# aksiksi/needle

Measured on AMD Instinct MI355X. Metric: episode-pairs/sec (analyze+search), higher is better.
Workload: dtype f64-certified (f32 first pass)

## Files before the change

needle_amd/csrc/search.hip:

```cpp
#include "epilogue.h"
#include "hipctx.h"

#include <algorithm>
#include <atomic>
#include <cstdio>
#include <cstdlib>
#include <cstring>
#include <mutex>
#include <unordered_map>

namespace needle {

namespace {

constexpr int kDiagsPerBlock = 256;
constexpr int kBandR = 7, kBandU = 3;
constexpr int kBandB = 64 * kBandR;
constexpr int kSampleW = 8;
constexpr int kSampleHead = 3;
__host__ __device__ constexpr int head_row(int k, int W, int H = kSampleHead) {
  return H == 3 ? (k == 0 ? 0 : (k == 1 ? W / 2 : W - 1)) : (k * (W - 1)) / (H - 1);
}
__host__ __device__ constexpr bool is_head_row(int s, int W, int H = kSampleHead) {
  for (int k = 0; k < H; k++)
// ... 99 lines not shown
  const int D0 = band * B - (n - 2);
  if (D0 > m - 2) return;
  const int i_start = max(1, 2 - D0 - B);
  const int i_end = min(n - 1, m - 1 - D0);
  if (i_start > i_end) return;
  const int d_l = D0 + lane * R;
  const int min_len = (int)pr.min_len;
  const int flag_len = min_len - K + 1;

  uint32_t W[R];
  int Z[R];
#pragma unroll
  for (int r = 0; r < R; r++) {
    W[r] = lds[B + i_start + d_l + r];
    Z[r] = i_start - 1;
  }

  auto checkpoint = [&](int c) {
#pragma unroll
    for (int r = 0; r < R; r++) {
      if (c - Z[r] >= flag_len) {
        const int d = d_l + r;
        const int ilo = d < 0 ? 1 - d : 1;
        const int ihi = min(n - 1, m - 1 - d);
        if (c >= ilo && c <= ihi) {
          const int a = max(Z[r] + 1, ilo);
          const int limit = min(ihi, c + K);
          int e = c + 1;
          while (e <= limit && (uint32_t)__popc(src[e] ^ lds[B + e + d]) <= threshold) e++;
          const bool reaches_next_checkpoint = (e > limit) && (limit == c + K);
          if (!reaches_next_checkpoint) {
            const int b = e - 1;
            const int len = b - a + 1;
            if (len >= min_len) {
              const uint32_t slot = atomicAdd(count, 1u);
              if (slot < capacity) runs[slot] = NeedleHipRun{(uint32_t)lo, (uint32_t)b, (uint32_t)(b + d), (uint32_t)len, 0u, 0u};
            }
          }
        }
      }
    }
  };

  int i = i_start;
  for (; i + K - 1 <= i_end; i += K) {
    const uint32_t *__restrict__ nxt = lds + (B + i + d_l + R);
#pragma unroll
    for (int s = 0; s < K; s++) {
      const int row = i + s;
      const uint32_t sv = src[row];
#pragma unroll
      for (int r = 0; r < R; r++) {
        const uint32_t c = (uint32_t)__popc(sv ^ W[(r + s) % R]);
        Z[r] = (c <= threshold) ? Z[r] : row;
        if (r == 0) W[s % R] = nxt[s];
      }
    }
    bool any = false;
#pragma unroll
    for (int r = 0; r < R; r++) any |= (i + K - 1 - Z[r] >= flag_len);
    if (__any(any)) checkpoint(i + K - 1);
  }
  for (; i <= i_end; i++) {
    const uint32_t sv = src[i];
#pragma unroll
    for (int r = 0; r < R; r++) {
      const uint32_t c = (uint32_t)__popc(sv ^ W[r]);
      Z[r] = (c <= threshold) ? Z[r] : i;
    }
#pragma unroll
    for (int r = 0; r + 1 < R; r++) W[r] = W[r + 1];
    W[R - 1] = lds[B + i + d_l + R];
  }
}

__device__ __forceinline__ void wave_lds_fence_search() {
  __builtin_amdgcn_fence(__ATOMIC_RELEASE, "wavefront");
  __builtin_amdgcn_wave_barrier();
  __builtin_amdgcn_fence(__ATOMIC_ACQUIRE, "wavefront");
}

template <int R, int W, bool COUNT = false, int H = kSampleHead, bool LEGACY = false>
__global__ __launch_bounds__(256) void hamming_runs_sampled_kernel(const uint32_t *__restrict__ hashes,
                                                                   const SearchProblem *__restrict__ problems,
                                                                   int num_problems, uint32_t threshold,
                                                                   NeedleHipRun *__restrict__ runs,
                                                                   uint32_t capacity, uint32_t *__restrict__ count,
                                                                   int bands_per_wave, int sparse_max,
                                                                   unsigned long long *__restrict__ eval_groups) {
  constexpr int B = 64 * R;
  unsigned long long groups = 0, survived = 0;
  extern __shared__ uint32_t lds[];
  __builtin_amdgcn_s_setprio(3);
  int lo = 0, hi = num_problems - 1;
  while (lo < hi) {
    int mid = (lo + hi + 1) >> 1;
    if (problems[mid].block_base <= blockIdx.x) lo = mid; else hi = mid - 1;
  }
  const SearchProblem pr = problems[lo];
  const int n = (int)pr.n, m = (int)pr.m;
  const uint32_t *__restrict__ src = hashes + pr.src_off;
  const uint32_t *__restrict__ dst = hashes + pr.dst_off;
  uint32_t *ldst = lds;
  for (int k = threadIdx.x; k < B; k += blockDim.x) {
    ldst[k] = 0u;
    ldst[B + m + k] = 0u;
  }
  {
    constexpr int kU = 8;
    const int nt = (int)blockDim.x;
    int k = threadIdx.x;
    for (; k + (kU - 1) * nt < m; k += kU * nt) {
      uint32_t v[kU];
#pragma unroll
      for (int u = 0; u < kU; u++) v[u] = dst[k + u * nt];
#pragma unroll
      for (int u = 0; u < kU; u++) ldst[B + k + u * nt] = v[u];
    }
    for (; k < m; k += nt) ldst[B + k] = dst[k];
  }
  const uint32_t *__restrict__ lsrc = src;
  __syncthreads();

  const int wave = __builtin_amdgcn_readfirstlane((int)(threadIdx.x >> 6));
  const int lane = (int)(threadIdx.x & 63);
  const int min_len = (int)pr.min_len;
  const int P = min_len - W + 1;
  const uint32_t bias = 31u - min(threshold, 31u);
  uint32_t held_b = 0u, held_e = 0u, held_len = 0u;
  int held = 0;
  auto flush_runs = [&]() {
    if (held == 0) return;
    uint32_t base = 0u;
    if (lane == 0) base = atomicAdd(count, (uint32_t)held);
    base = (uint32_t)__builtin_amdgcn_readfirstlane((int)base);
    if (lane < held && base + (uint32_t)lane < capacity)
      runs[base + (uint32_t)lane] = NeedleHipRun{(uint32_t)lo, held_b, held_e, held_len, 0u, 0u};
    held = 0;
  };
  auto emit_run = [&](const uint32_t b, const uint32_t e, const uint32_t len) {
    const bool mine = lane == held;
    held_b = mine ? b : held_b;
    held_e = mine ? e : held_e;
    held_len = mine ? len : held_len;
    if (++held == 64) flush_runs();
  };
  const int slots = 4 * bands_per_wave;
  const int total_bands = (n + m - 3 + B - 1) / B;
  const int nb = (total_bands + slots - 1) / slots;
  const int b_in_pair = (int)(blockIdx.x - pr.block_base);
  for (int round = 0; round < bands_per_wave; round++) {
  const int q = (round * 4 + wave + lo) % slots;
  const int band = q * nb + b_in_pair;
  const int D0 = band * B - (n - 2);
  if (band >= total_bands || D0 > m - 2) continue;
  const int i_start = max(1, 2 - D0 - B);
  const int i_end = min(n - 1, m - 1 - D0);
  const int d_l = D0 + lane * R;

  int k0 = (i_start - 1 + P - 1) / P;
  for (int w0 = 1 + k0 * P; w0 + W - 1 <= i_end; w0 += P) {
    uint32_t E[W + R - 1];
#pragma unroll
    for (int q = 0; q < W + R - 1; q++) E[q] = ldst[B + w0 + d_l + q];
    uint32_t sv[W];
#pragma unroll
    for (int s = 0; s < W; s++) sv[s] = src[w0 + s];
    bool ok[R];
    uint32_t miss[R];
#pragma unroll
    for (int r = 0; r < R; r++) miss[r] = 0u;
#pragma unroll
    for (int k = 0; k < H; k++) {
      const int s = head_row(k, W, H);
#pragma unroll
      for (int r = 0; r < R; r++) miss[r] |= (uint32_t)__popc(sv[s] ^ E[s + r]) + bias;
    }
#pragma unroll
    for (int r = 0; r < R; r++) ok[r] = miss[r] < 32u;
    if (COUNT) groups += H * R;
    auto resolve = [&](const int d) {
      const int ilo = d < 0 ? 1 - d : 1;
      const int ihi = min(n - 1, m - 1 - d);
      if (w0 < ilo || w0 + W - 1 > ihi) return;
      int e = w0 + W;
      bool ended = false;
      const int fwd_limit = min(ihi, w0 + P + W - 1);
      while (e <= fwd_limit) {
        const int row = e + lane;
        const bool bad = row <= fwd_limit && (uint32_t)__popc(lsrc[row] ^ ldst[B + row + d]) > threshold;
        if (COUNT) groups += 1;
        const unsigned long long mm = __ballot(bad);
        if (mm) {
          e += __ffsll((long long)mm) - 1;
          ended = true;
          break;
        }
        e += 64;
      }
      if (!ended) {
        if (fwd_limit == w0 + P + W - 1) return;
        e = ihi + 1;
      }
      const int b = e - 1;
      int a = ilo;
      int q = w0 - 1;
      while (q >= ilo) {
        const int row = q - lane;
        const bool bad = row >= ilo && (uint32_t)__popc(lsrc[row] ^ ldst[B + row + d]) > threshold;
        if (COUNT) groups += 1;
        const unsigned long long mm = __ballot(bad);
        if (mm) {
          a = q - (__ffsll((long long)mm) - 1) + 1;
          break;
        }
        q -= 64;
      }
      const int len = b - a + 1;
      if (len >= min_len) emit_run((uint32_t)b, (uint32_t)(b + d), (uint32_t)len);
    };

    unsigned long long alive[R];
    int survivors = 0;
#pragma unroll
    for (int r = 0; r < R; r++) {
      alive[r] = __ballot(ok[r]);
      survivors += __popcll(alive[r]);
    }
    if (COUNT) survived += (unsigned long long)survivors;
    if (survivors == 0) continue;
    if (!LEGACY || sparse_max < 0) {
#pragma unroll
      for (int r = 0; r < R; r++) {
        if (alive[r] == 0) continue;
        uint32_t mm = miss[r];
#pragma unroll
        for (int k = 0; k < W - H; k++) {
          const int s = tail_row(k, W, H);
          mm |= (uint32_t)__popc(sv[s] ^ E[s + r]) + bias;
        }
        if (COUNT) groups += W - H;
        unsigned long long cand = __ballot(mm < 32u);
        while (cand) {
          const int src_lane = __ffsll((long long)cand) - 1;
          cand &= cand - 1;
          resolve(D0 + src_lane * R + r);
        }
      }
      continue;
    }
    if constexpr (LEGACY) {
    if (survivors <= sparse_max) {
      constexpr int kTail = W - H;
      uint32_t sv_tail = sv[tail_row(kTail - 1, W, H)];
      int tail_off = tail_row(kTail - 1, W, H);
#pragma unroll
      for (int k = kTail - 2; k >= 0; k--) {
        sv_tail = lane == k ? sv[tail_row(k, W, H)] : sv_tail;
        tail_off = lane == k ? tail_row(k, W, H) : tail_off;
      }
#pragma unroll
      for (int r = 0; r < R; r++) {
        unsigned long long cand = alive[r];
        while (cand) {
          const int src_lane = __ffsll((long long)cand) - 1;
          cand &= cand - 1;
          const int d = D0 + src_lane * R + r;
          const int row = w0 + tail_off;
          const bool bad = (uint32_t)__popc(sv_tail ^ ldst[B + row + d]) > threshold;
          if (COUNT) groups += 1;
          if (__ballot(bad) == 0) resolve(d);
        }
      }
      continue;
    }
#pragma unroll
    for (int k = 0; k < W - H; k++) {
      const int s = tail_row(k, W, H);
#pragma unroll
      for (int r = 0; r < R; r++) miss[r] |= (uint32_t)__popc(sv[s] ^ E[s + r]) + bias;
    }
#pragma unroll
    for (int r = 0; r < R; r++) ok[r] = miss[r] < 32u;
    if (COUNT) groups += (W - H) * R;
#pragma unroll
    for (int r = 0; r < R; r++) {
      unsigned long long cand = __ballot(ok[r]);
      while (cand) {
        const int src_lane = __ffsll((long long)cand) - 1;
        cand &= cand - 1;
        resolve(D0 + src_lane * R + r);
      }
    }
    }
  }
  }
  flush_runs();
  if (COUNT && lane == 0) {
    atomicAdd(eval_groups, groups);
    atomicAdd(eval_groups + 1, survived);
  }
}

__host__ __device__ constexpr int mfma_windows(int n, int min_len, int W) {
  return (n - 1 - W) >= 0 && min_len - W + 1 > 0 ? (n - 1 - W) / (min_len - W + 1) + 1 : 0;
}
typedef int mfma_v4i __attribute__((ext_vector_type(4)));
typedef int mfma_v8i __attribute__((ext_vector_type(8)));
typedef float mfma_v16f __attribute__((ext_vector_type(16)));

#include "scan_mfma_kernel.h"

struct TransposeLane {
  uint32_t rot[5], mask[5];
};
__device__ __forceinline__ TransposeLane transpose_lane(uint32_t lane) {
  TransposeLane t;
  uint32_t m = 0x0000FFFFu;
#pragma unroll
  for (int k = 0; k < 5; k++) {
    const uint32_t j = 16u >> k;
    const bool hi = (lane & j) != 0u;
    t.rot[k] = hi ? 32u - j : j;
    t.mask[k] = hi ? m << j : m;
    m ^= m << (j >> 1);
  }
  return t;
}
template <int PATTERN>
__device__ __forceinline__ uint32_t swizzle_xor(uint32_t x) {
  return (uint32_t)__builtin_amdgcn_ds_swizzle((int)x, PATTERN);
}
__device__ __forceinline__ uint32_t transpose32(uint32_t x, const TransposeLane &t) {
#define NEEDLE_TSTEP(K, J)                                                              \
  {                                                                                     \
    const uint32_t y = swizzle_xor<((J) << 10) | 0x1F>(x);                              \
    const uint32_t r = __builtin_amdgcn_alignbit(y, y, t.rot[K]);                      \
    x = (r & t.mask[K]) | (x & ~t.mask[K]);                                             \
  }
  NEEDLE_TSTEP(0, 16) NEEDLE_TSTEP(1, 8) NEEDLE_TSTEP(2, 4) NEEDLE_TSTEP(3, 2) NEEDLE_TSTEP(4, 1)
#undef NEEDLE_TSTEP
  return x;
}
__device__ __forceinline__ uint32_t wave_simhash32(const uint32_t *__restrict__ slice, uint32_t count, uint32_t lane, const TransposeLane &t) {
  constexpr int kBlocks = 8;
  uint32_t ones = 0;
  for (uint32_t q0 = 0; q0 < count; q0 += 64 * kBlocks) {
    uint32_t h[kBlocks];
#pragma unroll
    for (int u = 0; u < kBlocks; u++) {
      const uint32_t q = q0 + 64 * u + lane;
      h[u] = q < count ? slice[q] : 0u;
    }
#pragma unroll
    for (int u = 0; u < kBlocks; u++) {
      if (q0 + 64 * u >= count) break;
      ones += (uint32_t)__popc(transpose32(h[u], t));
    }
  }
  ones += (uint32_t)__shfl_xor((int)ones, 32);
  const unsigned long long set = __builtin_amdgcn_ballot_w64(2u * ones > count);
  return __brev((uint32_t)set);
}

__global__ __launch_bounds__(256) void simhash_runs_kernel(const uint32_t *__restrict__ hashes,
                                                           const SearchProblem *__restrict__ problems,
                                                           NeedleHipRun *__restrict__ runs, uint32_t capacity,
                                                           const uint32_t *__restrict__ count) {
  const uint32_t total = min(*count, capacity);
  const uint32_t wave = (blockIdx.x * blockDim.x + threadIdx.x) >> 6, waves = (gridDim.x * blockDim.x) >> 6;
  const uint32_t lane = threadIdx.x & 63;
  __builtin_amdgcn_s_setprio(3);
  const TransposeLane t = transpose_lane(lane);
  for (uint32_t k = wave; k < total; k += waves) {
    const NeedleHipRun r = runs[k];
    const SearchProblem pr = problems[r.problem];
    const uint32_t src_hash = wave_simhash32(hashes + pr.src_off + (r.src_end - r.len), r.len + 1u, lane, t);
    const uint32_t dst_hash = wave_simhash32(hashes + pr.dst_off + (r.dst_end - r.len), r.len + 1u, lane, t);
    if (lane == 0) {
      runs[k].problem = pr.tag;
      runs[k].src_match_hash = src_hash;
      runs[k].dst_match_hash = dst_hash;
    }
  }
}

struct ScanShape {
  int w = kSampleW, h = kSampleHead;
};
ScanShape scan_shape() {
  ScanShape sh;
  if (const char *e = getenv("NEEDLE_HIP_SCAN_SHAPE")) {
    int w = 0, h = 0;
    if (std::sscanf(e, "%d,%d", &w, &h) == 2 && (w == 4 || w == 8 || w == 16) && h >= 2 && h <= 4 && h < w) {
      sh.w = w;
      sh.h = h;
    }
  }
  return sh;
}
using SampledKernel = void (*)(const uint32_t *, const SearchProblem *, int, uint32_t, NeedleHipRun *, uint32_t, uint32_t *, int, int,
                               unsigned long long *);
template <bool COUNT>
SampledKernel sampled_kernel(ScanShape sh, bool legacy) {
#define NEEDLE_SHAPE(W_, H_) \
  if (sh.w == W_ && sh.h == H_) return hamming_runs_sampled_kernel<kBandR, W_, COUNT, H_, true>;
  NEEDLE_SHAPE(4, 2) NEEDLE_SHAPE(4, 3) NEEDLE_SHAPE(8, 2) NEEDLE_SHAPE(8, 4) NEEDLE_SHAPE(16, 2) NEEDLE_SHAPE(16, 3) NEEDLE_SHAPE(16, 4)
#undef NEEDLE_SHAPE
  if (legacy) return hamming_runs_sampled_kernel<kBandR, kSampleW, COUNT, kSampleHead, true>;
  return hamming_runs_sampled_kernel<kBandR, kSampleW, COUNT, kSampleHead, false>;
}

struct SearchPlan {
  std::vector<NeedleHipSeq> seqs;
  std::vector<NeedleHipProblem> problems;
  int mode[8] = {0, 0, 0, 0, 0, 0, 0, 0};
  std::vector<SearchProblem> meta;
  size_t staged = 0;
  uint64_t oversize_blocks = 0;
  uint64_t blocks = 0;
  size_t lds_bytes = 0;
  bool sampled = false, fast = false, mfma = false;
  int mfma_waves = 0, mfma_splits = 1;
  std::vector<M2ImageSeq> image_seqs;
  uint32_t image_windows = 0, image_min_len = 0;
  uint64_t mfma_products = 0;
  int bands_per_wave = 1;
  bool valid = false;
  bool matches(const NeedleHipSeq *s, size_t ns, const NeedleHipProblem *p, size_t np, const int *m) const {
    return valid && seqs.size() == ns && problems.size() == np && std::memcmp(mode, m, sizeof(mode)) == 0 &&
           std::memcmp(seqs.data(), s, ns * sizeof(NeedleHipSeq)) == 0 &&
           std::memcmp(problems.data(), p, np * sizeof(NeedleHipProblem)) == 0;
  }
};

int device_cus() {
  int cus = 256, dev = 0;
  if (hipGetDevice(&dev) == hipSuccess) (void)hipDeviceGetAttribute(&cus, hipDeviceAttributeMultiprocessorCount, dev);
  return cus > 0 ? cus : 256;
}

Status build_plan(const NeedleHipSeq *seqs, size_t num_seqs, const NeedleHipProblem *problems, size_t num_problems,
                  const int *mode, SearchPlan *plan) {
  plan->valid = false;
  std::vector<SearchProblem> &meta = plan->meta;
  meta.clear();
  meta.reserve(num_problems);
  uint64_t blocks = 0;
  for (size_t p = 0; p < num_problems; p++) {
    const NeedleHipProblem &pr = problems[p];
    if (pr.src_seq >= num_seqs || pr.dst_seq >= num_seqs)
      return Status::Make(NeedleError_InvalidArgument, "hamming_runs: problem references a missing sequence");
    if (pr.min_len == 0) return Status::Make(NeedleError_InvalidArgument, "hamming_runs: min_len must be >= 1");
    const NeedleHipSeq &a = seqs[pr.src_seq], &b = seqs[pr.dst_seq];
    if (a.len < 2 || b.len < 2) continue;
    SearchProblem m;
    m.src_off = a.offset;
    m.n = a.len;
    m.dst_off = b.offset;
    m.m = b.len;
    m.min_len = pr.min_len;
    m.tag = pr.tag;
    m.block_base = 0;
    m.pad = 0;
    meta.push_back(m);
  }
  plan->staged = 0;
  plan->oversize_blocks = 0;
  if (!meta.empty()) {
    uint32_t smallest = 0xFFFFFFFFu;
    for (const SearchProblem &m : meta) smallest = std::min(smallest, m.min_len);
    const bool generic_only = mode[0] != 0;
    const bool sampled = !generic_only && smallest >= (uint32_t)(2 * scan_shape().w - 1 + 8) && mode[1] == 0 && mode[3] == 0;
    const bool fast = !generic_only && !sampled && smallest >= (uint32_t)(kBandR * kBandU);
    const size_t lds_limit = (size_t)mode[5];
    auto windows_of = [&](const SearchProblem &m) { return (uint64_t)mfma_windows((int)m.n, (int)m.min_len, kSampleW); };
    auto same_group = [](const SearchProblem &a, const SearchProblem &b) {
      return a.dst_off == b.dst_off && a.m == b.m && a.min_len == b.min_len;
    };
    const int waves = mode[6];
    const size_t group_budget = waves == 4 ? 53760 : waves == 8 ? 81920 : 163840;
    const size_t max_members = (size_t)kM2Members;
    auto group_need = [&](const SearchProblem &a, uint64_t windows) { return m2_lds_words(a.m, windows, waves) * sizeof(uint32_t); };
    bool mfma = sampled && mode[4] == 1;
    const size_t mfma_from = 2048;
    const bool candidate = sampled && (mode[4] == 1 || (mode[4] == 2 && meta.size() >= mfma_from));
    if (candidate) {
      std::stable_sort(meta.begin(), meta.end(), [](const SearchProblem &a, const SearchProblem &b) {
        if (a.dst_off != b.dst_off) return a.dst_off < b.dst_off;
        if (a.m != b.m) return a.m < b.m;
        return a.min_len < b.min_len;
      });
      if (!mfma) {
        uint64_t windows = 0, rows = 0;
        for (size_t i = 0; i < meta.size(); i++) {
          uint64_t w = windows_of(meta[i]);
          for (size_t k = 1; k < max_members && i + 1 < meta.size() && same_group(meta[i], meta[i + 1]) &&
                             group_need(meta[i], w + windows_of(meta[i + 1])) <= group_budget; k++)
            w += windows_of(meta[++i]);
          windows += w;
          rows += (w + 31) / 32 * 32;
        }
        mfma = rows > 0 && 10 * windows >= 7 * rows;
      }
    }
    auto lds_need = [&](const SearchProblem &m) {
      if (mfma) return group_need(m, windows_of(m));
      return ((fast || sampled) ? (size_t)m.m + 2 * kBandB : (size_t)m.n + m.m) * sizeof(uint32_t);
    };
    auto mfma_packable = [&](const SearchProblem &m) { return m.m < 65536u && windows_of(m) < 8192u && m.n < (1u << 28); };
    auto stageable = [&](const SearchProblem &m) { return lds_need(m) <= lds_limit && (!mfma || mfma_packable(m)); };
    std::stable_partition(meta.begin(), meta.end(), stageable);
    size_t staged = 0;
    while (staged < meta.size() && stageable(meta[staged])) staged++;
    size_t lds_bytes = 0;
    int bands_per_wave = 1;
    size_t groups = 0;
    if (mfma) {
      const bool single = (mode[7] & 0x100) != 0;
      for (size_t i = 0; i < staged;) {
        SearchProblem &a = meta[i];
        a.pad = 0;
        uint64_t windows = windows_of(a);
        size_t k = 1;
        while (!single && k < max_members && i + k < staged && same_group(a, meta[i + k]) &&
               windows + windows_of(meta[i + k]) < 8192 &&
               group_need(a, windows + windows_of(meta[i + k])) <= group_budget) {
          windows += windows_of(meta[i + k]);
          meta[i + k].pad = 0x80000000u;
          k++;
        }
        a.pad = (uint32_t)(k - 1);
        i += k;
        groups++;
      }
    }
    if (mfma) {
      if (staged >= ((size_t)1 << 23)) return Status::Make(NeedleError_InvalidArgument, "hamming_runs: too many problems for one launch");
      size_t g = 0;
      for (size_t i = 0; i < staged; i++)
        if (!(meta[i].pad & 0x80000000u)) meta[g++].pad |= (uint32_t)i << 8;
    }
    int splits = 1;
    if (mfma && groups > 0) {
      const uint64_t slots = (uint64_t)device_cus() * (uint64_t)(waves == 4 ? 3 : waves == 8 ? 2 : 1);
      splits = (int)std::min<uint64_t>(8, std::max<uint64_t>(1, (2 * slots + groups - 1) / groups));
      if (mode[7] & 0x7F) splits = mode[7] & 0x7F;
    }
    if (fast || sampled) {
      uint64_t fb = 0, total_bands = 0;
      for (size_t i = 0; i < staged; i++) total_bands += ((uint64_t)meta[i].n + meta[i].m - 3 + kBandB - 1) / kBandB;
      if (sampled)
        while (bands_per_wave < 8 && total_bands / (4 * (uint64_t)bands_per_wave * 2) >= 16384) bands_per_wave *= 2;
      if (mode[2] > 0) bands_per_wave = mode[2];
      for (size_t i = 0; i < staged; i++) {
        SearchProblem &m = meta[i];
        m.block_base = (uint32_t)fb;
        if (mfma && (m.pad & 0x80000000u)) continue;
        const uint64_t diags = (uint64_t)m.n + m.m - 3;
        const uint64_t bands = (diags + kBandB - 1) / kBandB;
        const uint64_t per_block = 4 * (uint64_t)(sampled ? bands_per_wave : 1);
        fb += mfma ? (uint64_t)splits : (bands + per_block - 1) / per_block;
        if (mfma) {
          uint64_t windows = windows_of(m);
          for (uint32_t f = 1; f <= (m.pad & 0xFFu); f++) windows += windows_of(meta[i + f]);
          lds_bytes = std::max(lds_bytes, group_need(m, windows));
        } else {
          lds_bytes = std::max(lds_bytes, lds_need(m));
        }
      }
      blocks = fb;
    } else {
      for (size_t i = 0; i < staged; i++) {
        SearchProblem &m = meta[i];
        m.block_base = (uint32_t)blocks;
        blocks += ((uint64_t)m.n + m.m - 3 + kDiagsPerBlock - 1) / kDiagsPerBlock;
        lds_bytes = std::max(lds_bytes, lds_need(m));
      }
    }
    uint64_t ob = 0;
    for (size_t i = staged; i < meta.size(); i++) {
      meta[i].block_base = (uint32_t)ob;
      ob += ((uint64_t)meta[i].n + meta[i].m - 3 + kDiagsPerBlock - 1) / kDiagsPerBlock;
    }
    if (blocks > 0x7FFFFFFFull || ob > 0x7FFFFFFFull)
      return Status::Make(NeedleError_InvalidArgument, "hamming_runs: too many problems for one launch");
    plan->staged = staged;
    plan->oversize_blocks = ob;
    plan->sampled = sampled;
    plan->mfma = mfma;
    plan->mfma_products = 0;
    if (mfma)
      for (size_t i = 0; i < staged; i++) {
        const SearchProblem &m = meta[i];
        if (m.pad & 0x80000000u) continue;
        uint64_t w = windows_of(m);
        for (uint32_t f = 1; f <= (m.pad & 0xFFu); f++) w += windows_of(meta[i + f]);
        if (w > 0 && m.m >= (uint32_t)kSampleW + 1) {
          uint64_t col_blocks = ((uint64_t)m.m - kSampleW) / 32 + 1;
          col_blocks = (col_blocks + kM2ColBlocks - 1) / kM2ColBlocks * kM2ColBlocks;
          plan->mfma_products += (w + 31) / 32 * col_blocks * (kM2Heads / 2);
        }
      }
    plan->image_seqs.clear();
    plan->image_windows = plan->image_min_len = 0;
    if (mfma && staged > 0 && !(mode[7] & 0x200)) {
      bool one = true;
      for (size_t i = 1; i < staged && one; i++) one = meta[i].min_len == meta[0].min_len;
      if (one) {
        std::unordered_map<uint64_t, uint32_t> first_of;
        uint64_t total = 0;
        for (size_t i = 0; i < staged; i++) {
          const uint64_t key = ((uint64_t)meta[i].src_off << 32) | meta[i].n;
          auto it = first_of.find(key);
          if (it == first_of.end()) {
            const uint32_t w = (uint32_t)windows_of(meta[i]);
            it = first_of.emplace(key, (uint32_t)total).first;
            plan->image_seqs.push_back(M2ImageSeq{meta[i].src_off, meta[i].n, (uint32_t)total, w});
            total += w;
          }
          meta[i].block_base = it->second;
        }
        if (total == 0 || total * kM2ImageWords * sizeof(uint32_t) > ((uint64_t)1 << 31)) {
          plan->image_seqs.clear();
        } else {
          plan->image_windows = (uint32_t)total;
          plan->image_min_len = meta[0].min_len;
        }
      }
    }
    plan->fast = fast;
    plan->mfma_waves = waves;
    plan->mfma_splits = splits;
    plan->bands_per_wave = bands_per_wave;
    plan->lds_bytes = lds_bytes;
  }
  plan->blocks = blocks;
  plan->seqs.assign(seqs, seqs + num_seqs);
  plan->problems.assign(problems, problems + num_problems);
  std::memcpy(plan->mode, mode, sizeof(plan->mode));
  plan->valid = true;
  return Status::Ok();
}

int mfma_request(uint32_t threshold) {
  if (threshold > 15u || scan_shape().w != kSampleW || getenv("NEEDLE_HIP_SCAN_SHAPE") || getenv("NEEDLE_HIP_SCAN_COUNT")) return 0;
  const char *e = getenv("NEEDLE_HIP_SCAN_MFMA");
  if (!e) return 2;
  return atoi(e) != 0 ? 1 : 0;
}

int mfma_waves() {
  int waves = 8;
  if (const char *e = getenv("NEEDLE_HIP_MFMA_WAVES")) {
    const int w = atoi(e);
    if (w == 4 || w == 8 || w == 12 || w == 16) waves = w;
  }
  return waves;
}
using Mfma2Kernel = void (*)(const uint32_t *, const SearchProblem *, int, uint32_t, NeedleHipRun *, uint32_t, uint32_t *, int, const uint32_t *);
Mfma2Kernel mfma2_kernel(int waves) {
  return waves == 4 ? hamming_runs_mfma2_kernel<kSampleW, 4, 3> : waves == 16 ? hamming_runs_mfma2_kernel<kSampleW, 16, 4>
       : waves == 12 ? hamming_runs_mfma2_kernel<kSampleW, 12, 3> : hamming_runs_mfma2_kernel<kSampleW, 8, 4>;
}

std::atomic<int32_t> g_last_form{0};
std::atomic<uint64_t> g_last_products{0};

struct SearchWorkspace {
  DeviceBuffer<SearchProblem> problems;
  PinnedStage stage;
  DescriptorUpload<SearchProblem> upload;
  SearchPlan plan;
  DeviceBuffer<M2ImageSeq> image_seqs;
  PinnedStage image_stage;
  DescriptorUpload<M2ImageSeq> image_upload;
  DeviceBuffer<uint32_t> images;
  bool lds_attr_set = false;
  unsigned long long *eval_groups = nullptr;
};
std::mutex g_ws_mu;
std::map<int, SearchWorkspace *> g_ws;

SearchWorkspace *workspace() {
  int dev = 0;
  (void)hipGetDevice(&dev);
  std::lock_guard<std::mutex> lock(g_ws_mu);
  auto it = g_ws.find(dev);
  if (it != g_ws.end()) return it->second;
  SearchWorkspace *w = new SearchWorkspace();
  g_ws[dev] = w;
  return w;
}


}

void gpu_scan_last_launch(int32_t *form, uint64_t *matrix_products) {
  *form = g_last_form.load();
  *matrix_products = g_last_products.load();
}

Status gpu_hamming_runs_device(const uint32_t *d_hashes, const NeedleHipSeq *seqs, size_t num_seqs,
                               const NeedleHipProblem *problems, size_t num_problems, uint32_t threshold,
                               NeedleHipRun *d_runs, uint32_t capacity, uint32_t *d_count, bool sync, bool count_is_zero) {
  std::lock_guard<std::recursive_mutex> gpu_lock(gpu_mutex());
  Status s = ensure_device();
  if (!s.ok()) return s;
  hipStream_t stream = library_stream();
  if (!count_is_zero) NEEDLE_HIP_TRY(hipMemsetAsync(d_count, 0, sizeof(uint32_t), stream));
  const int mode[8] = {getenv("NEEDLE_HIP_GENERIC_SEARCH") != nullptr, getenv("NEEDLE_HIP_BAND_SEARCH") != nullptr,
                       getenv("NEEDLE_HIP_BANDS_PER_WAVE") ? std::max(1, atoi(getenv("NEEDLE_HIP_BANDS_PER_WAVE"))) : 0,
                       threshold > 31u,
                       mfma_request(threshold),
                       getenv("NEEDLE_HIP_SEARCH_LDS_LIMIT") ? std::max(1, atoi(getenv("NEEDLE_HIP_SEARCH_LDS_LIMIT"))) : 160 * 1024,
                       mfma_waves(),
                       (getenv("NEEDLE_HIP_MFMA_SPLITS") ? std::max(1, std::min(64, atoi(getenv("NEEDLE_HIP_MFMA_SPLITS")))) : 0) |
                           (getenv("NEEDLE_HIP_MFMA_SINGLE") ? 0x100 : 0) | (getenv("NEEDLE_HIP_MFMA_NO_IMAGES") ? 0x200 : 0)};
  SearchWorkspace *ws = workspace();
  SearchPlan &plan = ws->plan;
  const bool reuse = plan.matches(seqs, num_seqs, problems, num_problems, mode);
  if (!reuse && !(s = build_plan(seqs, num_seqs, problems, num_problems, mode, &plan)).ok()) return s;
  const std::vector<SearchProblem> &meta = plan.meta;
  const uint64_t blocks = plan.blocks;
  const size_t lds_bytes = plan.lds_bytes;
  const bool sampled = plan.sampled, fast = plan.fast;
  const int bands_per_wave = plan.bands_per_wave;
  if (!meta.empty()) {
    if (!(reuse && ws->upload.resident_at == ws->problems.ptr && ws->problems.ptr) &&
        !(s = ws->upload.put(&ws->problems, &ws->stage, meta, stream)).ok())
      return s;
    if (lds_bytes > 64 * 1024 && !ws->lds_attr_set) {
      NEEDLE_HIP_TRY(hipFuncSetAttribute(reinterpret_cast<const void *>(hamming_runs_kernel<true>),
                                         hipFuncAttributeMaxDynamicSharedMemorySize, 160 * 1024));
      NEEDLE_HIP_TRY(hipFuncSetAttribute(reinterpret_cast<const void *>(hamming_runs_band_kernel<kBandR, kBandU>),
                                         hipFuncAttributeMaxDynamicSharedMemorySize, 160 * 1024));
      for (int w : {4, 8, 12, 16})
        NEEDLE_HIP_TRY(hipFuncSetAttribute(reinterpret_cast<const void *>(mfma2_kernel(w)),
                                           hipFuncAttributeMaxDynamicSharedMemorySize, 160 * 1024));
      for (int w : {4, 8, 16})
        for (int h : {2, 3, 4}) {
          if (h >= w) continue;
          for (bool legacy : {false, true}) {
            NEEDLE_HIP_TRY(hipFuncSetAttribute(reinterpret_cast<const void *>(sampled_kernel<false>(ScanShape{w, h}, legacy)),
                                               hipFuncAttributeMaxDynamicSharedMemorySize, 160 * 1024));
            NEEDLE_HIP_TRY(hipFuncSetAttribute(reinterpret_cast<const void *>(sampled_kernel<true>(ScanShape{w, h}, legacy)),
                                               hipFuncAttributeMaxDynamicSharedMemorySize, 160 * 1024));
          }
        }
      ws->lds_attr_set = true;
    }
    const int staged = (int)plan.staged, oversize = (int)(meta.size() - plan.staged);
    g_last_form.store(staged > 0 ? (sampled ? (plan.mfma ? 4 : 3) : fast ? 2 : 1) : 1);
    g_last_products.store(staged > 0 && plan.mfma ? plan.mfma_products : 0);
    if (staged > 0) {
      KernelTimer timer("hamming_runs");
      if (sampled) {
        int sparse_max = -1;
        if (const char *e = getenv("NEEDLE_HIP_SPARSE_MAX")) sparse_max = std::max(0, atoi(e));
        if (getenv("NEEDLE_HIP_SCAN_COUNT")) {
          if (!ws->eval_groups) {
            NEEDLE_HIP_TRY(hipMalloc((void **)&ws->eval_groups, 2 * sizeof(unsigned long long)));
            NEEDLE_HIP_TRY(hipMemsetAsync(ws->eval_groups, 0, 2 * sizeof(unsigned long long), stream));
          }
          hipLaunchKernelGGL(sampled_kernel<true>(scan_shape(), sparse_max >= 0), dim3((uint32_t)blocks), dim3(256), lds_bytes, stream, d_hashes,
                             ws->problems.ptr, staged, threshold, d_runs, capacity, d_count, bands_per_wave, sparse_max,
                             ws->eval_groups);
        } else if (plan.mfma) {
          const uint32_t *images = nullptr;
          if (!plan.image_seqs.empty()) {
            if (!(s = ws->image_upload.put(&ws->image_seqs, &ws->image_stage, plan.image_seqs, stream)).ok() ||
                !(s = ws->images.reserve((size_t)plan.image_windows * kM2ImageWords)).ok())
              return s;
            const uint32_t grid = (uint32_t)std::min<uint64_t>(8192, ((uint64_t)plan.image_windows * kM2Rows + 255) / 256);
            hipLaunchKernelGGL(m2_window_images_kernel<kSampleW>, dim3(grid), dim3(256), 0, stream, d_hashes, ws->image_seqs.ptr,
                               (int)plan.image_seqs.size(), plan.image_windows, plan.image_min_len, ws->images.ptr);
            images = ws->images.ptr;
          }
          hipLaunchKernelGGL(mfma2_kernel(plan.mfma_waves), dim3((uint32_t)blocks), dim3(64 * plan.mfma_waves),
                             lds_bytes, stream, d_hashes, ws->problems.ptr, staged, threshold, d_runs, capacity, d_count,
                             plan.mfma_splits, images);
#if NEEDLE_M2_LAB & 8
          {
            unsigned long long c[8], z[8] = {};
            (void)hipStreamSynchronize(stream);
            (void)hipMemcpyFromSymbol(c, HIP_SYMBOL(m2_dbg), sizeof c);
            (void)hipMemcpyToSymbol(HIP_SYMBOL(m2_dbg), z, sizeof z);
            fprintf(stderr, "m2 counts: resolve calls %llu, trips %llu, mismatches handled %llu, walks continued %llu, extra forward trips %llu, "
                            "windows past the tail rows %llu, items %llu, windows past the head rows %llu\n", c[0], c[1], c[2], c[3], c[4], c[5], c[6], c[7]);
          }
#endif
        } else {
          hipLaunchKernelGGL(sampled_kernel<false>(scan_shape(), sparse_max >= 0), dim3((uint32_t)blocks), dim3(256), lds_bytes, stream, d_hashes,
                             ws->problems.ptr, staged, threshold, d_runs, capacity, d_count, bands_per_wave, sparse_max,
                             (unsigned long long *)nullptr);
        }
      }
      else if (fast)
        hipLaunchKernelGGL((hamming_runs_band_kernel<kBandR, kBandU>), dim3((uint32_t)blocks), dim3(256), lds_bytes,
                           stream, d_hashes, ws->problems.ptr, staged, threshold, d_runs, capacity, d_count);
      else
        hipLaunchKernelGGL(hamming_runs_kernel<true>, dim3((uint32_t)blocks), dim3(256), lds_bytes, stream, d_hashes,
                           ws->problems.ptr, staged, 0u, threshold, d_runs, capacity, d_count);
    }
    if (oversize > 0) {
      KernelTimer timer("hamming_runs_unstaged");
      hipLaunchKernelGGL(hamming_runs_kernel<false>, dim3((uint32_t)plan.oversize_blocks), dim3(256), 0, stream, d_hashes,
                         ws->problems.ptr + staged, oversize, (uint32_t)staged, threshold, d_runs, capacity, d_count);
    }
    {
      KernelTimer timer("simhash_runs");
      hipLaunchKernelGGL(simhash_runs_kernel, dim3(2048), dim3(256), 0, stream, d_hashes, ws->problems.ptr, d_runs,
                         capacity, d_count);
    }
    NEEDLE_HIP_TRY(hipGetLastError());
  }
  if (sync) NEEDLE_HIP_TRY(hipStreamSynchronize(stream));
  return Status::Ok();
}

Status gpu_scan_issued_evaluations(uint64_t *lane_evaluations, bool reset, uint64_t *head_survivors) {
  std::lock_guard<std::recursive_mutex> gpu_lock(gpu_mutex());
  Status s = ensure_device();
  if (!s.ok()) return s;
  SearchWorkspace *ws = workspace();
  unsigned long long groups[2] = {0, 0};
  hipStream_t stream = library_stream();
  if (ws->eval_groups) {
    NEEDLE_HIP_TRY(hipMemcpyAsync(groups, ws->eval_groups, sizeof(groups), hipMemcpyDeviceToHost, stream));
    if (reset) NEEDLE_HIP_TRY(hipMemsetAsync(ws->eval_groups, 0, sizeof(groups), stream));
    NEEDLE_HIP_TRY(hipStreamSynchronize(stream));
  }
  *lane_evaluations = (uint64_t)groups[0] * 64u;
  if (head_survivors) *head_survivors = (uint64_t)groups[1];
  return Status::Ok();
}

namespace {
struct HostCallBuffers {
  DeviceBuffer<uint32_t> d_hashes, d_count;
  DeviceBuffer<NeedleHipRun> d_runs;
  void *pinned = nullptr;
  size_t pinned_bytes = 0;
  uint32_t *arena = nullptr;
  size_t arena_words = 0;
  bool arena_out = false;
  const uint32_t *sent = nullptr;
  size_t sent_words = 0;
};
HostCallBuffers *host_call_buffers() {
  static std::map<int, HostCallBuffers *> all;
  int dev = 0;
  (void)hipGetDevice(&dev);
  HostCallBuffers *&hb = all[dev];
  if (!hb) hb = new HostCallBuffers();
  return hb;
}
}

uint32_t *gpu_pinned_arena_acquire(size_t words) {
  std::lock_guard<std::recursive_mutex> gpu_lock(gpu_mutex());
  if (!ensure_device().ok()) return nullptr;
  HostCallBuffers *hb = host_call_buffers();
  if (hb->arena_out || getenv("NEEDLE_HIP_PAGEABLE_ARENA")) return nullptr;
  if (words > hb->arena_words) {
    if (hb->arena) (void)hipHostFree(hb->arena);
    hb->arena = nullptr;
    hb->arena_words = 0;
    void *p = nullptr;
    const size_t want = words + words / 8 + 1024;
    if (hipHostMalloc(&p, want * sizeof(uint32_t), hipHostMallocDefault) != hipSuccess) {
      (void)hipGetLastError();
      return nullptr;
    }
    hb->arena = static_cast<uint32_t *>(p);
    hb->arena_words = want;
  }
  hb->arena_out = true;
  return hb->arena;
}
void gpu_pinned_arena_release(uint32_t *p) {
  if (!p) return;
  std::lock_guard<std::recursive_mutex> gpu_lock(gpu_mutex());
  HostCallBuffers *hb = host_call_buffers();
  if (hb->sent) (void)hipStreamSynchronize(library_stream());
  hb->sent = nullptr;
  hb->arena_out = false;
}
void gpu_prefetch_hashes(const uint32_t *hashes, size_t num_hashes) {
  std::lock_guard<std::recursive_mutex> gpu_lock(gpu_mutex());
  if (!ensure_device().ok()) return;
  HostCallBuffers *hb = host_call_buffers();
  hb->sent = nullptr;
  if (hashes != hb->arena || !hb->arena_out || num_hashes == 0) return;
  if (!hb->d_hashes.reserve(num_hashes).ok()) return;
  if (hipMemcpyAsync(hb->d_hashes.ptr, hashes, num_hashes * sizeof(uint32_t), hipMemcpyHostToDevice, library_stream()) != hipSuccess) {
    (void)hipGetLastError();
    return;
  }
  hb->sent = hashes;
  hb->sent_words = num_hashes;
}
namespace {
Status upload_hashes(HostCallBuffers *hb, const uint32_t *hashes, size_t num_hashes, hipStream_t stream) {
  const bool sent = hb->sent == hashes && hb->sent_words == num_hashes && num_hashes > 0;
  hb->sent = nullptr;
  if (!sent) NEEDLE_HIP_TRY(hipMemcpyAsync(hb->d_hashes.ptr, hashes, num_hashes * sizeof(uint32_t), hipMemcpyHostToDevice, stream));
  return Status::Ok();
}
}

Status gpu_search_results_host(const uint32_t *hashes, size_t num_hashes, const NeedleHipSeq *seqs, size_t num_seqs,
                               const NeedleHipProblem *problems, size_t num_problems, uint32_t threshold, EpilogueJob job,
                               std::vector<NeedleHipSearchResult> *results, uint32_t *failed, std::vector<NeedleHipRun> *runs,
                               size_t *num_runs) {
  std::lock_guard<std::recursive_mutex> gpu_lock(gpu_mutex());
  Status s = ensure_device();
  if (!s.ok()) return s;
  for (size_t i = 0; i < num_seqs; i++)
    if ((uint64_t)seqs[i].offset + seqs[i].len > num_hashes)
      return Status::Make(NeedleError_InvalidArgument, "hamming_runs: sequence outside the hash arena");
  hipStream_t stream = library_stream();
  HostCallBuffers *hb = host_call_buffers();
  if (!(s = hb->d_hashes.reserve(std::max<size_t>(num_hashes, 1))).ok() || !(s = hb->d_count.reserve(1)).ok()) return s;
  const size_t want = ((size_t)job.n + 1) * sizeof(NeedleHipSearchResult);
  if (want > hb->pinned_bytes) {
    if (hb->pinned) (void)hipHostFree(hb->pinned);
    hb->pinned = nullptr;
    hb->pinned_bytes = 0;
    NEEDLE_HIP_TRY(hipHostMalloc(&hb->pinned, want, hipHostMallocDefault));
    hb->pinned_bytes = want;
  }
  NeedleHipSearchResult *pinned = static_cast<NeedleHipSearchResult *>(hb->pinned);
  uint32_t *pinned_failed = reinterpret_cast<uint32_t *>(pinned + job.n);
  if (!(s = upload_hashes(hb, hashes, num_hashes, stream)).ok()) return s;
  uint32_t capacity = (uint32_t)std::min<uint64_t>(
      0x7fffffffu, std::max<uint64_t>({(uint64_t)1 << 16, (uint64_t)hb->d_runs.count, 3 * (uint64_t)num_problems}));
  for (int attempt = 0; attempt < 2; attempt++) {
    if (!(s = hb->d_runs.reserve(capacity)).ok()) return s;
    s = gpu_hamming_runs_device(hb->d_hashes.ptr, seqs, num_seqs, problems, num_problems, threshold, hb->d_runs.ptr, capacity,
                                hb->d_count.ptr, false, false);
    if (!s.ok()) return s;
    uint32_t found = 0;
    NEEDLE_HIP_TRY(hipMemcpyAsync(&found, hb->d_count.ptr, sizeof(found), hipMemcpyDeviceToHost, stream));
    NEEDLE_HIP_TRY(hipStreamSynchronize(stream));
    if (found <= capacity) {
      job.num_segments = 1;
      job.segment_count[0] = hb->d_count.ptr;
      job.segment_runs[0] = hb->d_runs.ptr;
      job.segment_capacity = capacity;
      job.max_runs = (uint64_t)found + (found >> 3) + 1024;
      if (!(s = gpu_epilogue_enqueue(job, stream, pinned, pinned_failed)).ok()) return s;
      NEEDLE_HIP_TRY(hipStreamSynchronize(stream));
      *num_runs = found;
      *failed = *pinned_failed;
      results->assign(pinned, pinned + job.n);
      runs->clear();
      if (*failed && found) {
        runs->resize(found);
        NEEDLE_HIP_TRY(hipMemcpy(runs->data(), hb->d_runs.ptr, found * sizeof(NeedleHipRun), hipMemcpyDeviceToHost));
      }
      return Status::Ok();
    }
    capacity = found;
  }
  return Status::Make(NeedleError_Unknown, "hamming_runs: run list did not fit after resize");
}

Status gpu_hamming_runs_host(const uint32_t *hashes, size_t num_hashes, const NeedleHipSeq *seqs, size_t num_seqs,
                             const NeedleHipProblem *problems, size_t num_problems, uint32_t threshold,
                             std::vector<NeedleHipRun> *runs) {
  std::lock_guard<std::recursive_mutex> gpu_lock(gpu_mutex());
  Status s = ensure_device();
  if (!s.ok()) return s;
  for (size_t i = 0; i < num_seqs; i++)
    if ((uint64_t)seqs[i].offset + seqs[i].len > num_hashes)
      return Status::Make(NeedleError_InvalidArgument, "hamming_runs: sequence outside the hash arena");
  hipStream_t stream = library_stream();
  HostCallBuffers *hb = host_call_buffers();
  DeviceBuffer<uint32_t> &d_hashes = hb->d_hashes, &d_count = hb->d_count;
  DeviceBuffer<NeedleHipRun> &d_runs = hb->d_runs;
  if (!(s = d_hashes.reserve(std::max<size_t>(num_hashes, 1))).ok()) return s;
  if (!(s = d_count.reserve(1)).ok()) return s;
  if (!(s = upload_hashes(hb, hashes, num_hashes, stream)).ok()) return s;
  uint32_t capacity = (uint32_t)std::min<uint64_t>(
      0x7fffffffu, std::max<uint64_t>({(uint64_t)1 << 16, (uint64_t)d_runs.count, 3 * (uint64_t)num_problems}));
  for (int attempt = 0; attempt < 2; attempt++) {
    if (!(s = d_runs.reserve(capacity)).ok()) return s;
    s = gpu_hamming_runs_device(d_hashes.ptr, seqs, num_seqs, problems, num_problems, threshold, d_runs.ptr,
                                capacity, d_count.ptr, false, false);
    if (!s.ok()) return s;
    uint32_t found = 0;
    NEEDLE_HIP_TRY(hipMemcpyAsync(&found, d_count.ptr, sizeof(found), hipMemcpyDeviceToHost, stream));
    NEEDLE_HIP_TRY(hipStreamSynchronize(stream));
    if (found <= capacity) {
      runs->resize(found);
      if (found)
        NEEDLE_HIP_TRY(hipMemcpy(runs->data(), d_runs.ptr, found * sizeof(NeedleHipRun), hipMemcpyDeviceToHost));
      return Status::Ok();
    }
    capacity = found;
  }
  return Status::Make(NeedleError_Unknown, "hamming_runs: run list did not fit after resize");
}

namespace {
template <int R>
__global__ __launch_bounds__(256) void valu_ceiling_sampled_kernel(uint32_t *out, int rows, uint32_t threshold, uint32_t seed) {
  uint32_t Wd[R + 2];
#pragma unroll
  for (int r = 0; r < R + 2; r++) Wd[r] = seed * (threadIdx.x + 1) * (r + 3) + blockIdx.x;
  const uint32_t bias = 31u - threshold;
  uint32_t sv = __builtin_amdgcn_readfirstlane(seed ^ blockIdx.x);
  int total = 0;
  for (int i = 0; i < rows; i += 3) {
    uint32_t s0 = sv * 1664525u + 1013904223u, s1 = s0 * 1664525u + 1013904223u, s2 = s1 * 1664525u + 1013904223u;
    sv = s2;
    int survivors = 0;
#pragma unroll
    for (int r = 0; r < R; r++) {
      const uint32_t miss = ((uint32_t)__popc(s0 ^ Wd[r]) + bias) | ((uint32_t)__popc(s1 ^ Wd[r + 1]) + bias) |
                            ((uint32_t)__popc(s2 ^ Wd[r + 2]) + bias);
      survivors += __popcll(__ballot(miss < 32u));
    }
    total += survivors;
    if (survivors == (int)seed) Wd[0] ^= 1u;
  }
  out[blockIdx.x * blockDim.x + threadIdx.x] = (uint32_t)total + Wd[0];
}

template <int R>
__global__ __launch_bounds__(256) void valu_ceiling_kernel(uint32_t *out, int rows, uint32_t threshold, uint32_t seed) {
  uint32_t W[R];
  int Z[R];
#pragma unroll
  for (int r = 0; r < R; r++) {
    W[r] = seed * (threadIdx.x + 1) * (r + 3) + blockIdx.x;
    Z[r] = -1;
  }
  uint32_t sv = __builtin_amdgcn_readfirstlane(seed ^ blockIdx.x);
  for (int i = 0; i < rows; i++) {
    sv = sv * 1664525u + 1013904223u;
#pragma unroll
    for (int r = 0; r < R; r++) {
      const uint32_t c = (uint32_t)__popc(sv ^ W[r]);
      Z[r] = (c <= threshold) ? Z[r] : i;
    }
  }
  uint32_t acc = 0;
#pragma unroll
  for (int r = 0; r < R; r++) acc += (uint32_t)Z[r];
  out[blockIdx.x * blockDim.x + threadIdx.x] = acc;
}
}

Status gpu_int_valu_ceiling(double *cells_per_second) {
  std::lock_guard<std::recursive_mutex> gpu_lock(gpu_mutex());
  Status s = ensure_device();
  if (!s.ok()) return s;
  constexpr int R = 8;
// ... 45 lines not shown
```

Measured before the change: 713,100.

## Add comb-tooth sampled search kernel using spaced anchor rows and bit-packed match masks

Adds a new search kernel that samples source 'teeth' every min_len/2 rows and, for each destination column, builds a bitmask of which teeth match within threshold. It stores these masks in LDS and finds candidates where consecutive teeth both match. Candidates are pre-filtered with three interior probes before a full forward and backward run resolution. The aim is to replace dense diagonal band scanning with a sparse anchor-based search. This is enabled by default when sampled and not MFMA. It adds a per-problem work split, extra LDS usage and serialized per-candidate resolution cost.

```diff
diff --git a/needle_amd/csrc/scan_comb_kernel.h b/needle_amd/csrc/scan_comb_kernel.h
--- /dev/null
+++ b/needle_amd/csrc/scan_comb_kernel.h
@@ -0,0 +1,183 @@
+
+constexpr int kCombQ = 4;
+constexpr int kCombMaxPairs = 31;
+constexpr int kCombStack = 128;
+constexpr int kCombMaxWords = 11776;
+constexpr uint32_t kCombMaxS = 2048;
+
+__host__ __device__ constexpr size_t comb_lds_bytes(int lds_words) { return ((size_t)lds_words + 4 * kCombStack) * sizeof(uint32_t); }
+
+template <bool COUNT>
+__global__ __launch_bounds__(256) __attribute__((amdgpu_num_vgpr(32)))
+void hamming_runs_comb_kernel(const uint32_t *__restrict__ hashes, const SearchProblem *__restrict__ problems, int num_problems,
+                              uint32_t threshold, NeedleHipRun *__restrict__ runs, uint32_t capacity, uint32_t *__restrict__ count,
+                              int lds_words, unsigned long long *__restrict__ eval_groups) {
+  constexpr int Q = kCombQ;
+  unsigned long long groups = 0, survived = 0;
+  extern __shared__ uint32_t lds[];
+  __builtin_amdgcn_s_setprio(3);
+  int lo = 0, hi = num_problems - 1;
+  while (lo < hi) {
+    int mid = (lo + hi + 1) >> 1;
+    if (problems[mid].block_base <= blockIdx.x) lo = mid; else hi = mid - 1;
+  }
+  const SearchProblem pr = problems[lo];
+  const int n = (int)pr.n, m = (int)pr.m;
+  const uint32_t *__restrict__ src = hashes + pr.src_off;
+  const uint32_t *__restrict__ dst = hashes + pr.dst_off;
+  const int min_len = (int)pr.min_len;
+  const int s = min_len >> 1;
+  const int K = (n - 1) / s;
+  const int kb = 1 + (int)(blockIdx.x - pr.block_base) * (int)pr.pad;
+  if (K < 2 || kb >= K || m - 1 <= s) return;
+  const int T = min((int)pr.pad, K - kb) + 1;
+  const int wave = __builtin_amdgcn_readfirstlane((int)(threadIdx.x >> 6));
+  const int lane = (int)(threadIdx.x & 63);
+  uint32_t *mm = lds;
+  uint32_t *stack = lds + lds_words + wave * kCombStack;
+  const uint32_t tooth_hash = src[(kb + min(lane, T - 1)) * s];
+  const uint32_t bias = 0x7FFFFFFFu - min(threshold, 31u);
+
+  uint32_t held_b = 0u, held_e = 0u, held_len = 0u;
+  int held = 0;
+  auto flush_runs = [&]() {
+    if (held == 0) return;
+    uint32_t base = 0u;
+    if (lane == 0) base = atomicAdd(count, (uint32_t)held);
+    base = (uint32_t)__builtin_amdgcn_readfirstlane((int)base);
+    if (lane < held && base + (uint32_t)lane < capacity)
+      runs[base + (uint32_t)lane] = NeedleHipRun{(uint32_t)lo, held_b, held_e, held_len, 0u, 0u};
+    held = 0;
+  };
+  auto emit_run = [&](const uint32_t b, const uint32_t e, const uint32_t len) {
+    const bool mine = lane == held;
+    held_b = mine ? b : held_b;
+    held_e = mine ? e : held_e;
+    held_len = mine ? len : held_len;
+    if (++held == 64) flush_runs();
+  };
+
+  auto resolve = [&](const int r, const int d) {
+    const int ilo = d < 0 ? 1 - d : 1;
+    const int ihi = min(n - 1, m - 1 - d);
+    for (int row0 = r + 1; row0 < r + s; row0 += 64) {
+      const int row = row0 + lane;
+      const bool bad = row < r + s && (uint32_t)__popc(src[row] ^ dst[row + d]) > threshold;
+      if (COUNT) groups += 1;
+      if (__ballot(bad)) return;
+    }
+    int e = r + s + 1;
+    bool ended = false;
+    const int fwd_limit = min(ihi, r + 2 * s);
+    while (e <= fwd_limit) {
+      const int row = e + lane;
+      const bool bad = row <= fwd_limit && (uint32_t)__popc(src[row] ^ dst[row + d]) > threshold;
+      if (COUNT) groups += 1;
+      const unsigned long long mmask = __ballot(bad);
+      if (mmask) {
+        e += __ffsll((long long)mmask) - 1;
+        ended = true;
+        break;
+      }
+      e += 64;
+    }
+    if (!ended) {
+      if (fwd_limit == r + 2 * s) return;
+      e = ihi + 1;
+    }
+    const int b = e - 1;
+    int a = ilo;
+    int q = r - 1;
+    while (q >= ilo) {
+      const int row = q - lane;
+      const bool bad = row >= ilo && (uint32_t)__popc(src[row] ^ dst[row + d]) > threshold;
+      if (COUNT) groups += 1;
+      const unsigned long long mmask = __ballot(bad);
+      if (mmask) {
+        a = q - (__ffsll((long long)mmask) - 1) + 1;
+        break;
+      }
+      q -= 64;
+    }
+    const int len = b - a + 1;
+    if (len >= min_len) emit_run((uint32_t)b, (uint32_t)(b + d), (uint32_t)len);
+  };
+
+  const int p1 = s >> 2, p2 = s >> 1, p3 = (3 * s) >> 2;
+  auto take = [&](const uint32_t *from, const int cnt, const int c0) {
+    wave_lds_fence_search();
+    const bool act = lane < cnt;
+    const uint32_t entry = act ? from[lane] : 0u;
+    wave_lds_fence_search();
+    const int r = act ? (kb + T - 1 - (int)(entry & 31u)) * s : 0;
+    const int j = act ? c0 + (int)(entry >> 5) : 0;
+    const uint32_t a1 = src[r + p1], a2 = src[r + p2], a3 = src[r + p3];
+    const uint32_t b1 = dst[j + p1], b2 = dst[j + p2], b3 = dst[j + p3];
+    const bool ok = act && (uint32_t)__popc(a1 ^ b1) <= threshold && (uint32_t)__popc(a2 ^ b2) <= threshold &&
+                    (uint32_t)__popc(a3 ^ b3) <= threshold;
+    if (COUNT) groups += 3;
+    unsigned long long surv = __ballot(ok);
+    while (surv) {
+      const int l = __ffsll((long long)surv) - 1;
+      surv &= surv - 1;
+      const int ru = __builtin_amdgcn_readlane(r, l), ju = __builtin_amdgcn_readlane(j, l);
+      resolve(ru, ju - ru);
+    }
+  };
+
+  const int step = lds_words - s;
+  for (int c0 = 1; c0 + s < m; c0 += step) {
+    const int jend = min(c0 + lds_words, m);
+    for (int blk = c0 + wave * (64 * Q); blk < jend; blk += 4 * 64 * Q) {
+      uint32_t E[Q], acc[Q];
+#pragma unroll
+      for (int q = 0; q < Q; q++) {
+        const int j = blk + q * 64 + lane;
+        E[q] = j < jend ? dst[j] : 0u;
+        acc[q] = 0xFFFFFFFFu;
+      }
+      for (int t = 0; t < T; t++) {
+        const uint32_t sv = (uint32_t)__builtin_amdgcn_readlane((int)tooth_hash, t);
+#pragma unroll
+        for (int q = 0; q < Q; q++) acc[q] = __builtin_amdgcn_alignbit(acc[q], (uint32_t)__popc(sv ^ E[q]) + bias, 31u);
+      }
+      if (COUNT) groups += (unsigned long long)(T * Q);
+#pragma unroll
+      for (int q = 0; q < Q; q++) {
+        const int j = blk + q * 64 + lane;
+        if (j < jend) mm[j - c0] = acc[q];
+      }
+    }
+    __syncthreads();
+    const int pend = min(c0 + step, m - s);
+    int fill = 0;
+    for (int blk = c0 + wave * 64; blk < pend; blk += 256) {
+      const int j = blk + lane;
+      uint32_t c = 0u;
+      if (j < pend) c = ~(mm[j - c0] | (mm[j + s - c0] << 1)) & ~1u;
+      unsigned long long has;
+      while ((has = __ballot(c != 0u)) != 0ull) {
+        if (c != 0u) {
+          const int bit = 31 - __clz((int)c);
+          const int pos = fill + (int)__builtin_amdgcn_mbcnt_hi((uint32_t)(has >> 32), __builtin_amdgcn_mbcnt_lo((uint32_t)has, 0u));
+          stack[pos] = ((uint32_t)(j - c0) << 5) | (uint32_t)bit;
+          c &= ~(1u << bit);
+        }
+        const int pushed = __popcll(has);
+        if (COUNT) survived += (unsigned long long)pushed;
+        fill += pushed;
+        if (fill >= 64) {
+          fill -= 64;
+          take(stack + fill, 64, c0);
+        }
+      }
+    }
+    if (fill > 0) take(stack, fill, c0);
+    __syncthreads();
+  }
+  flush_runs();
+  if (COUNT && lane == 0) {
+    atomicAdd(eval_groups, groups);
+    atomicAdd(eval_groups + 1, survived);
+  }
+}
diff --git a/needle_amd/csrc/search.hip b/needle_amd/csrc/search.hip
--- a/needle_amd/csrc/search.hip
+++ b/needle_amd/csrc/search.hip
@@ -425,6 +425,8 @@
   }
 }
 
+#include "scan_comb_kernel.h"
+
 __host__ __device__ constexpr int mfma_windows(int n, int min_len, int W) {
   return (n - 1 - W) >= 0 && min_len - W + 1 > 0 ? (n - 1 - W) / (min_len - W + 1) + 1 : 0;
 }
@@ -537,13 +539,14 @@
 struct SearchPlan {
   std::vector<NeedleHipSeq> seqs;
   std::vector<NeedleHipProblem> problems;
-  int mode[8] = {0, 0, 0, 0, 0, 0, 0, 0};
+  int mode[9] = {0, 0, 0, 0, 0, 0, 0, 0, 0};
   std::vector<SearchProblem> meta;
   size_t staged = 0;
   uint64_t oversize_blocks = 0;
   uint64_t blocks = 0;
   size_t lds_bytes = 0;
-  bool sampled = false, fast = false, mfma = false;
+  bool sampled = false, fast = false, mfma = false, comb = false;
+  int comb_words = 0;
   int mfma_waves = 0, mfma_splits = 1;
   std::vector<M2ImageSeq> image_seqs;
   uint32_t image_windows = 0, image_min_len = 0;
@@ -638,6 +641,14 @@
     while (staged < meta.size() && stageable(meta[staged])) staged++;
     size_t lds_bytes = 0;
     int bands_per_wave = 1;
+    bool comb = sampled && !mfma && (mode[8] & 1) != 0 && staged > 0;
+    for (size_t i = 0; i < staged && comb; i++) comb = meta[i].min_len / 2 <= kCombMaxS;
+    int comb_words = 0;
+    if (comb) {
+      uint32_t longest = 0;
+      for (size_t i = 0; i < staged; i++) longest = std::max(longest, meta[i].m);
+      comb_words = (int)std::min<uint64_t>((uint64_t)kCombMaxWords, ((uint64_t)longest + 255) / 256 * 256);
+    }
     size_t groups = 0;
     if (mfma) {
       const bool single = (mode[7] & 0x100) != 0;
@@ -676,9 +687,19 @@
       if (sampled)
         while (bands_per_wave < 8 && total_bands / (4 * (uint64_t)bands_per_wave * 2) >= 16384) bands_per_wave *= 2;
       if (mode[2] > 0) bands_per_wave = mode[2];
+      const uint64_t comb_split = (mode[8] >> 4) > 0 ? (uint64_t)(mode[8] >> 4) : (staged < 1024 ? 4 : 1);
       for (size_t i = 0; i < staged; i++) {
         SearchProblem &m = meta[i];
         m.block_base = (uint32_t)fb;
+        if (comb) {
+          const uint64_t s = m.min_len / 2, teeth = ((uint64_t)m.n - 1) / s, pairs = teeth > 1 ? teeth - 1 : 1;
+          const uint64_t wgs = std::max(std::min(comb_split, pairs), (pairs + kCombMaxPairs - 1) / kCombMaxPairs);
+          const uint64_t per_wg = (pairs + wgs - 1) / wgs;
+          m.pad = (uint32_t)per_wg;
+          fb += (pairs + per_wg - 1) / per_wg;
+          lds_bytes = comb_lds_bytes(comb_words);
+          continue;
+        }
         if (mfma && (m.pad & 0x80000000u)) continue;
         const uint64_t diags = (uint64_t)m.n + m.m - 3;
         const uint64_t bands = (diags + kBandB - 1) / kBandB;
@@ -712,6 +733,8 @@
     plan->oversize_blocks = ob;
     plan->sampled = sampled;
     plan->mfma = mfma;
+    plan->comb = comb;
+    plan->comb_words = comb_words;
     plan->mfma_products = 0;
     if (mfma)
       for (size_t i = 0; i < staged; i++) {
@@ -787,6 +810,14 @@
        : waves == 12 ? hamming_runs_mfma2_kernel<kSampleW, 12, 3> : hamming_runs_mfma2_kernel<kSampleW, 8, 4>;
 }
 
+int comb_request() {
+  int want = !(getenv("NEEDLE_HIP_SCAN_SHAPE") || getenv("NEEDLE_HIP_SPARSE_MAX") || getenv("NEEDLE_HIP_BANDS_PER_WAVE"));
+  if (const char *e = getenv("NEEDLE_HIP_SCAN_COMB")) want = atoi(e) != 0;
+  int split = 0;
+  if (const char *e = getenv("NEEDLE_HIP_COMB_SPLIT")) split = std::max(1, std::min(1024, atoi(e)));
+  return want | (split << 4);
+}
+
 std::atomic<int32_t> g_last_form{0};
 std::atomic<uint64_t> g_last_products{0};
 
@@ -832,14 +863,15 @@
   if (!s.ok()) return s;
   hipStream_t stream = library_stream();
   if (!count_is_zero) NEEDLE_HIP_TRY(hipMemsetAsync(d_count, 0, sizeof(uint32_t), stream));
-  const int mode[8] = {getenv("NEEDLE_HIP_GENERIC_SEARCH") != nullptr, getenv("NEEDLE_HIP_BAND_SEARCH") != nullptr,
+  const int mode[9] = {getenv("NEEDLE_HIP_GENERIC_SEARCH") != nullptr, getenv("NEEDLE_HIP_BAND_SEARCH") != nullptr,
                        getenv("NEEDLE_HIP_BANDS_PER_WAVE") ? std::max(1, atoi(getenv("NEEDLE_HIP_BANDS_PER_WAVE"))) : 0,
                        threshold > 31u,
                        mfma_request(threshold),
                        getenv("NEEDLE_HIP_SEARCH_LDS_LIMIT") ? std::max(1, atoi(getenv("NEEDLE_HIP_SEARCH_LDS_LIMIT"))) : 160 * 1024,
                        mfma_waves(),
                        (getenv("NEEDLE_HIP_MFMA_SPLITS") ? std::max(1, std::min(64, atoi(getenv("NEEDLE_HIP_MFMA_SPLITS")))) : 0) |
-                           (getenv("NEEDLE_HIP_MFMA_SINGLE") ? 0x100 : 0) | (getenv("NEEDLE_HIP_MFMA_NO_IMAGES") ? 0x200 : 0)};
+                           (getenv("NEEDLE_HIP_MFMA_SINGLE") ? 0x100 : 0) | (getenv("NEEDLE_HIP_MFMA_NO_IMAGES") ? 0x200 : 0),
+                       comb_request()};
   SearchWorkspace *ws = workspace();
   SearchPlan &plan = ws->plan;
   const bool reuse = plan.matches(seqs, num_seqs, problems, num_problems, mode);
@@ -878,7 +910,19 @@
     g_last_products.store(staged > 0 && plan.mfma ? plan.mfma_products : 0);
     if (staged > 0) {
       KernelTimer timer("hamming_runs");
-      if (sampled) {
+      if (sampled && plan.comb) {
+        unsigned long long *groups = nullptr;
+        if (getenv("NEEDLE_HIP_SCAN_COUNT")) {
+          if (!ws->eval_groups) {
+            NEEDLE_HIP_TRY(hipMalloc((void **)&ws->eval_groups, 2 * sizeof(unsigned long long)));
+            NEEDLE_HIP_TRY(hipMemsetAsync(ws->eval_groups, 0, 2 * sizeof(unsigned long long), stream));
+          }
+          groups = ws->eval_groups;
+        }
+        hipLaunchKernelGGL(groups ? hamming_runs_comb_kernel<true> : hamming_runs_comb_kernel<false>, dim3((uint32_t)blocks), dim3(256),
+                           lds_bytes, stream, d_hashes, ws->problems.ptr, staged, threshold, d_runs, capacity, d_count,
+                           plan.comb_words, groups);
+      } else if (sampled) {
         int sparse_max = -1;
         if (const char *e = getenv("NEEDLE_HIP_SPARSE_MAX")) sparse_max = std::max(0, atoi(e));
         if (getenv("NEEDLE_HIP_SCAN_COUNT")) {
```

New measurement: 721,700 (median of 6 runs). No clear change (+1.2%).
